# RyanXLi/OneshotDet

Hardware: AMD Instinct MI355X
Metric: images/sec/GPU fwd+bwd, 800x1024 target + 127x127 query, bs=8; 1->8 GPU scaling (higher is better)
Workload: dtype bf16; 1 GPU; BASELINE.json configs[2]: bs=8/GPU, 800x1024 target + 127x127 query, bf16 MFMA convs, forward (two R-50-FPN backbones, query pooling, correlation, FCOS head, training proposals) + FCOS loss + backward (stem/layer1 frozen) + gradient all-reduce + SGD(momentum) + weight repack; global_batch=8, parallelism=dp1: one rank, no collective anywhere in the step, world_size=1

## Files before the change

oneshotdet_amd/_lib.py:

```python
import ctypes as C
import os

_HERE = os.path.dirname(os.path.abspath(__file__))
LIB_PATH = os.environ.get("OSD_LIB_PATH") or os.path.join(_HERE, "lib", "liboneshotdet_hip.so")

OSD_F32, OSD_BF16 = 0, 1
ABI_VERSION = 4
ACT_NONE, ACT_RELU, ACT_EXP_SCALE = 0, 1, 2
RES_NONE, RES_SAME, RES_UP2X, RES_DOWN2X = 0, 1, 2, 3
GN_SPLITS = 64


class ConvDesc(C.Structure):
    _fields_ = [(n, C.c_int32) for n in (
        "dtype", "n", "h", "w", "cin", "in_stride_n", "in_stride_h", "in_stride_w", "ho", "wo", "cout", "r", "s",
        "stride_h", "stride_w", "pad_h", "pad_w", "w_rows", "out_stride", "res_mode", "res_h", "res_w", "res_stride",
        "act")] + [("act_scale", C.c_float), ("relu_in", C.c_int32), ("algo", C.c_int32), ("reserved0", C.c_int32),
                   ("ordered_ws", C.c_void_p), ("ordered_ws_bytes", C.c_int64)]


_p, _i, _f, _i64 = C.c_void_p, C.c_int, C.c_float, C.c_int64

SIGNATURES = {
    "osd_last_error_string": (C.c_char_p, []),
# ... 79 lines not shown
    "osd_box_decode": (_i, [_p, _p, _p, _p, _p, _p, _p, _i, _i, _i, _i, _p, _f, _f, _p, _f, _i, _p]),
    "osd_append_gt_boxes": (_i, [_p, _p, _p, _p, _p, _p, _p, _p, _i, _i, _i, _p]),
    "osd_proposals_sort_nms": (_i, [_p, _p, _i, _i, _i, _p, _p, _i, _i, _f, _i, _i, _p, _p, _p, _p, _p]),
    "osd_proposals_sort_nms_hint": (_i, [_p, _p, _i, _i, _i, _p, _p, _i, _i, _f, _i, _i, _i, _p, _p, _p, _p, _p, _p]),
    "osd_proposals_workspace_bytes": (_i64, [_i, _i, _i, _i]),
    "osd_box_match_sample": (_i, [_p, _p, _p, _p, _p, _p, _i, _i, _i, _i, _f, _f, _p, _p, _p, _p, _p, _p, _p, _p, _p]),
    "osd_box_loss": (_i, [_p, _p, _p, _p, _i, _i, _i, _f, _f, _p, _p, _i, _i, _p]),
    "osd_voc_match": (_i, [_p, _p, _p, _p, _p, _p, _p, _p, _i, _i, _i, _f, _p, _p, _p]),
    "osd_voc_curves": (_i, [_p, _p, _p, _i, _p, _p, _p]),
    "osd_voc_ap": (_i, [_p, _p, _p, _p, _p, _i, _i, _p, _p]),
    "osd_coco_match": (_i, [_p, _p, _p, _p, _p, _p, _i, _i, _i, _p, _i, _p, _i, _p, _p, _p, _p]),
    "osd_groupnorm_act_rois_bwd": (_i, [_p, _p, _p, _p, _p, _p, _p, _p, _p, _i, _i, _i, _i, _f, _f, _i, _i, _i, _i, _p]),
    "osd_rois_sum": (_i, [_p, _p, _i, _i, _i64, _i, _p]),
    "osd_roi_pool_levels_bwd": (_i, [_i, _p, _p, _p, _p, _p, _p, _p, _i, _i, _i, _i, _i, _i, _i, _p]),
    "osd_image_transform": (_i, [_p, _i, _i, _i, _i, _i, _i, _p, _p, _p, _i, _i, _i, _i, _i, _i, _i, _p, _p]),
    "osd_image_transform_workspace_bytes": (_i64, [_i, _i, _i, _i]),
    "osd_image_transform_batch": (_i, [_i, _p, _p, _p, _p, _p, _p, _i, _p, _p, _p, _i, _i, _i, _i, _i, _i, _i, _p, _p]),
}

BOX_CLS_CE, BOX_CLS_FOCAL, BOX_CLS_MSE = 0, 1, 2
SIGNATURES_BOX_MODES = {
    "osd_box_loss_opt": (_i, [_p, _p, _p, _p, _i, _i, _i, _f, _f, _p, _p, _i, _i, _i, _f, _f, _p]),
    "osd_box_decode_opt": (_i, [_p, _p, _p, _p, _p, _p, _p, _i, _i, _i, _i, _p, _f, _f, _p, _f, _i, _i, _p]),
}

BOX_CLS_L1, BOX_CLS_CXE = 3, 4
SOFT_LABEL_DISCRETE, SOFT_LABEL_LINEAR, SOFT_LABEL_TRANS_LINEAR, SOFT_LABEL_TRANS_4TH_LINEAR = 0, 1, 2, 3
SIGNATURES_SOFT_LABELS = {
    "osd_box_match_sample_soft": (_i, [_p, _p, _p, _p, _p, _p, _i, _i, _i, _i, _f, _f, _p, _p, _p, _p, _p, _p, _p, _p, _i, _p, _p, _p]),
    "osd_box_loss_soft": (_i, [_p, _p, _p, _p, _i, _i, _i, _f, _f, _p, _p, _i, _i, _p, _i, _p]),
}

SIGNATURES_NEG_SUPPORT = {
    "osd_box_loss_neg_support": (_i, [_p, _p, _p, _p, _p, _i, _i, _i, _f, _f, _f, _f, _p, _p, _p, _i, _i, _p]),
}

SIGNATURES_SOLVER = {
    "osd_solver_set": (_i, [_p, _f, _i, _p]),
    "osd_sgd_momentum_multi_dev": (_i, [_p, _p, _i, _p, _p, _p, _p, _f, _p]),
    "osd_sgd_momentum_pack_multi_dev": (_i, [_p, _p, _i, _p, _p, _p, _p, _p, _i, _p, _f, _i, _p]),
}

SIGNATURES_CLASS_SWEEP = {
    "osd_class_sweep_group": (_i, []),
    "osd_correlate_levels_sweep": (_i, [_i, _p, _p, _p, _p, _i, _i, _i, _i, _p]),
    "osd_roi_pool_levels_sweep": (_i, [_i, _p, _p, _p, _p, _p, _p, _p, _i, _i, _i, _i, _i, _i, _i, _p, _i, _p]),
}

SIGNATURES_GALLERY = {
    "osd_correlate_levels_gallery": (_i, [_i, _p, _p, _p, _p, _p, _i, _i, _i, _i, _i, _p]),
    "osd_groupnorm_act_rois_gallery": (_i, [_p, _p, _p, _p, _p, _p, _i, _i, _i, _i, _f, _f, _i, _i, _i, _i, _i, _p]),
}

_lib = None


class OsdError(RuntimeError):
    pass


def load():
    global _lib
    if _lib is not None:
        return _lib
    if not os.path.exists(LIB_PATH):
        raise OsdError("liboneshotdet_hip.so not built (%s missing): run `python -m oneshotdet_amd.build` or "
                       "__graft_entry__.build(); there is no CPU/eager fallback" % LIB_PATH)
    import torch
    lib = C.CDLL(LIB_PATH)
    for name, (res, args) in (list(SIGNATURES.items()) + list(SIGNATURES_BOX_MODES.items()) + list(SIGNATURES_SOFT_LABELS.items())
                              + list(SIGNATURES_NEG_SUPPORT.items()) + list(SIGNATURES_SOLVER.items())
                              + list(SIGNATURES_CLASS_SWEEP.items()) + list(SIGNATURES_GALLERY.items())):
        fn = getattr(lib, name)
        fn.restype = res
        fn.argtypes = args
    if lib.osd_abi_version() != ABI_VERSION:
        raise OsdError("%s reports ABI %d, this binding is written for ABI %d: rebuild it (`python -m oneshotdet_amd.build`)"
                       % (LIB_PATH, lib.osd_abi_version(), ABI_VERSION))
    _lib = lib
    return lib


def check(rc, what=""):
    if rc != 0:
        msg = load().osd_last_error_string()
        err = OsdError("%s failed (%d): %s" % (what, rc, msg.decode() if msg else "?"))
        err.code = rc
        raise err


def call(name, *args):
    lib = load()
    check(getattr(lib, name)(*args), name)
```

oneshotdet_amd/build.py:

```python
import os
import subprocess
import sys

HERE = os.path.dirname(os.path.abspath(__file__))
CSRC = os.path.join(HERE, "csrc")
LIBDIR = os.path.join(HERE, "lib")
TAG = os.environ.get("OSD_BUILD_TAG", "")
LIB = os.path.join(LIBDIR, "liboneshotdet_hip%s.so" % ("_" + TAG if TAG else ""))
SOURCES = ["osd_error.hip", "conv_igemm.hip", "conv_igemm_dma.hip", "conv_igemm_sp.hip", "conv_pred.hip", "conv_px.hip", "conv_wgrad.hip", "conv_wgrad_sk.hip", "backward.hip", "groupnorm_onepass.hip", "loss.hip", "elementwise.hip", "proposals.hip", "box_head.hip", "transforms.hip", "box_train.hip", "evaluation.hip", "query_avgpool.hip", "class_sweep.hip", "gallery.hip"]
HIPCC = os.environ.get("HIPCC", "/opt/rocm/bin/hipcc")
FLAGS = ["--offload-arch=gfx950", "-O3", "-fPIC", "-std=c++17", "-Wno-unused-result"] + os.environ.get("OSD_BUILD_FLAGS", "").split()


def _stale(target, deps):
    if not os.path.exists(target):
        return True
    t = os.path.getmtime(target)
    return any(os.path.getmtime(d) > t for d in deps)


def build_library(force=False, verbose=True):
    os.makedirs(LIBDIR, exist_ok=True)
    objdir = os.path.join(LIBDIR, "obj" + ("_" + TAG if TAG else ""))
    os.makedirs(objdir, exist_ok=True)
    headers = sorted(os.path.join(CSRC, f) for f in os.listdir(CSRC) if f.endswith(".h")) + [os.path.join(os.path.dirname(HERE), "include", h) for h in ("oneshotdet_hip.h", "oneshotdet_hip_box_modes.h", "oneshotdet_hip_soft_labels.h", "oneshotdet_hip_neg_support.h", "oneshotdet_hip_solver.h", "oneshotdet_hip_class_sweep.h", "oneshotdet_hip_gallery.h")]
    keep = set(src.replace(".hip", ".o") for src in SOURCES)
    for f in os.listdir(objdir):
        if f.endswith(".o") and f not in keep:
            os.remove(os.path.join(objdir, f))
    objs, procs = [], []
    for src in SOURCES:
        s = os.path.join(CSRC, src)
        o = os.path.join(objdir, src.replace(".hip", ".o"))
        objs.append(o)
        if force or _stale(o, [s] + headers):
            cmd = [HIPCC] + FLAGS + ["-c", s, "-o", o]
            if verbose:
                print(" ".join(cmd), flush=True)
            procs.append((src, subprocess.Popen(cmd, stdout=subprocess.PIPE, stderr=subprocess.STDOUT)))
    for src, p in procs:
        out, _ = p.communicate()
        if p.returncode != 0:
            sys.stderr.write(out.decode())
            raise RuntimeError("hipcc failed on %s" % src)
    if force or procs or _stale(LIB, objs):
        cmd = [HIPCC, "--offload-arch=gfx950", "-shared", "-fPIC", "-o", LIB] + objs
        if verbose:
            print(" ".join(cmd), flush=True)
        subprocess.check_call(cmd)
    return LIB


if __name__ == "__main__":
    print(build_library(force="--force" in sys.argv))
```

oneshotdet_amd/csrc/backward.hip:

```cpp
#include "osd_common.h"
#include "conv_params.h"

namespace {

constexpr int kMaxBlocks = 2048;
inline int grid_for(long long work, int threads) {
  long long b = (work + threads - 1) / threads;
  if (b < 1) b = 1;
  return (int)(b > kMaxBlocks ? kMaxBlocks : b);
}

template <typename T> struct Chunk;
template <> struct Chunk<float> {
  static constexpr int N = 4;
  float v[4];
  __device__ __forceinline__ void load(const float* p) {
    const float4 t = *reinterpret_cast<const float4*>(p);
    v[0] = t.x; v[1] = t.y; v[2] = t.z; v[3] = t.w;
  }
  __device__ __forceinline__ void store(float* p) const { *reinterpret_cast<float4*>(p) = make_float4(v[0], v[1], v[2], v[3]); }
};
template <> struct Chunk<__bf16> {
  static constexpr int N = 8;
  float v[8];
  __device__ __forceinline__ void load(const __bf16* p) {
    const bf16x8 t = *reinterpret_cast<const bf16x8*>(p);
#pragma unroll
    for (int i = 0; i < 8; ++i) v[i] = (float)t[i];
  }
  __device__ __forceinline__ void store(__bf16* p) const {
    bf16x8 t;
#pragma unroll
    for (int i = 0; i < 8; ++i) t[i] = (__bf16)v[i];
    *reinterpret_cast<bf16x8*>(p) = t;
  }
};

template <typename T>
__global__ void pack_dgrad_weight_kernel(const float* __restrict__ w, const float* __restrict__ scale, T* __restrict__ dst,
                                         int cout, int cin, int R, int S, int rows, int cout_pad, int src_orsi) {
  const long long total = (long long)rows * R * S * cout_pad;
  for (long long i = blockIdx.x * (long long)blockDim.x + threadIdx.x; i < total; i += (long long)gridDim.x * blockDim.x) {
    const int co = (int)(i % cout_pad);
    long long t = i / cout_pad;
    const int s = (int)(t % S); t /= S;
    const int r = (int)(t % R);
    const int ci = (int)(t / R);
    float v = 0.f;
    if (co < cout && ci < cin) {
      v = src_orsi ? w[(((size_t)co * R + (R - 1 - r)) * S + (S - 1 - s)) * cin + ci]
                   : w[(((size_t)co * cin + ci) * R + (R - 1 - r)) * S + (S - 1 - s)];
      if (scale) v *= scale[co];
    }
    dst[i] = from_f32<T>(v);
// ... 93 lines not shown
      for (int j = 0; j < (64 * CPW) / 256; ++j) {
        const int idx = threadIdx.x + 256 * j;
        const int ci = ci0 + idx / CPW, cc = (idx % CPW) * EP;
        if (ci >= e.rows) continue;
        T* o = out + (((size_t)ci * e.R + rr) * e.S + ss) * e.kpad + co0 + cc;
        if constexpr (sizeof(T) == 2) {
          bf16x8 v;
#pragma unroll
          for (int q = 0; q < 8; ++q) v[q] = (__bf16)big[cc + q][idx / CPW];
          *reinterpret_cast<bf16x8*>(o) = v;
        } else {
          *reinterpret_cast<f32x4*>(o) = f32x4{big[cc][idx / CPW], big[cc + 1][idx / CPW], big[cc + 2][idx / CPW], big[cc + 3][idx / CPW]};
        }
      }
    }
    return;
  }
  __shared__ float tile[32][33];
  const int tx = threadIdx.x & 31, ty = threadIdx.x >> 5;
  const int tci = (e.rows + 31) / 32, tco = (e.kpad + 31) / 32;
  const int ntiles = e.R * e.S * tci * tco;
  for (int t = blockIdx.x - e.first_block; t < ntiles; t += e.n_blocks) {
    const int cot = t % tco;
    int u = t / tco;
    const int cit = u % tci; u /= tci;
    const int s = u % e.S, r = u / e.S;
    const int co0 = cot * 32, ci0 = cit * 32;
    __syncthreads();
#pragma unroll
    for (int j = 0; j < 4; ++j) {
      const int co = co0 + ty + 8 * j, ci = ci0 + tx;
      float v = 0.f;
      if (co < e.cout && ci < e.cin) {
        v = w[(((size_t)co * e.R + (e.R - 1 - r)) * e.S + (e.S - 1 - s)) * e.cin + ci];
        if (sc) v *= sc[co];
      }
      tile[ty + 8 * j][tx] = v;
    }
    __syncthreads();
#pragma unroll
    for (int j = 0; j < 4; ++j) {
      const int ci = ci0 + ty + 8 * j, co = co0 + tx;
      if (ci < e.rows && co < e.kpad) out[(((size_t)ci * e.R + r) * e.S + s) * e.kpad + co] = from_f32<T>(tile[tx][ty + 8 * j]);
    }
  }
}

struct SgdEntry {
  long long off, numel;
  float lr_mult, wd;
  int first_block, n_blocks;
};

__device__ __forceinline__ float sgd_update(float w, float g, float b, float wd, float momentum, float step, int first, float& m) {
  const float d = __builtin_fmaf(wd, w, g);
  m = first ? d : __builtin_fmaf(momentum, b, d);
  return __builtin_fmaf(-step, m, w);
}

struct alignas(8) SolverBlock { float lr; int first_step; };
static_assert(sizeof(SolverBlock) == 8, "solver block layout (oneshotdet_hip_solver.h)");

__global__ void __launch_bounds__(64) solver_set_kernel(SolverBlock* __restrict__ block, float lr, int first_step) {
  if (blockIdx.x == 0 && threadIdx.x == 0) { block->lr = lr; block->first_step = first_step; }
}

__device__ __forceinline__ void sgd_multi_body(const SgdEntry* __restrict__ table, const int* __restrict__ block_entry,
                                               float* __restrict__ p, const float* __restrict__ g,
                                               float* __restrict__ buf, float lr, float momentum, int first) {
  const SgdEntry e = table[block_entry[blockIdx.x]];
  const float step = lr * e.lr_mult;
  const long long stride = (long long)e.n_blocks * blockDim.x;
  const long long tid = (long long)(blockIdx.x - e.first_block) * blockDim.x + threadIdx.x;
  const long long n4 = (e.off & 3) == 0 ? (e.numel >> 2) : 0;
  f32x4* p4 = reinterpret_cast<f32x4*>(p + e.off);
  const f32x4* g4 = reinterpret_cast<const f32x4*>(g + e.off);
  f32x4* b4 = reinterpret_cast<f32x4*>(buf + e.off);
  for (long long i = tid; i < n4; i += stride) {
    const f32x4 w = p4[i], gr = g4[i];
    f32x4 bb = f32x4{0.f, 0.f, 0.f, 0.f};
    if (!first) bb = b4[i];
    f32x4 m, o;
#pragma unroll
    for (int k = 0; k < 4; ++k) { float mk; o[k] = sgd_update(w[k], gr[k], bb[k], e.wd, momentum, step, first, mk); m[k] = mk; }
    b4[i] = m;
    p4[i] = o;
  }
  for (long long i = n4 * 4 + tid; i < e.numel; i += stride) {
    const long long k = e.off + i;
    const float w = p[k];
    float m;
    const float o = sgd_update(w, g[k], first ? 0.f : buf[k], e.wd, momentum, step, first, m);
    buf[k] = m;
    p[k] = o;
  }
}

__global__ void __launch_bounds__(256) sgd_multi_kernel(const SgdEntry* __restrict__ table, const int* __restrict__ block_entry,
                                                        float* __restrict__ p, const float* __restrict__ g,
                                                        float* __restrict__ buf, float lr, float momentum, int first) {
  sgd_multi_body(table, block_entry, p, g, buf, lr, momentum, first);
}

__global__ void __launch_bounds__(256) sgd_multi_dev_kernel(const SgdEntry* __restrict__ table, const int* __restrict__ block_entry,
                                                            float* __restrict__ p, const float* __restrict__ g,
                                                            float* __restrict__ buf, const SolverBlock* __restrict__ solver,
                                                            float momentum) {
  const SolverBlock s = *solver;
  sgd_multi_body(table, block_entry, p, g, buf, s.lr, momentum, s.first_step);
}

struct SgdPackEntry {
  long long off, numel;
  float lr_mult, wd;
// ... 376 lines not shown
}

#define OSD_STREAM(s) reinterpret_cast<hipStream_t>(s)
#define OSD_DISPATCH_DTYPE(dtype, CALL_F32, CALL_BF16)                            \
  do {                                                                           \
    if ((dtype) == OSD_F32) { CALL_F32; }                                        \
    else if ((dtype) == OSD_BF16) { CALL_BF16; }                                 \
    else return osd_fail(OSD_ERR_INVALID_ARG, "bad dtype %d", (int)(dtype));     \
  } while (0)

extern "C" int osd_pack_conv_weight_dgrad(const float* w, const float* scale, void* dst, int cout, int cin, int r, int s,
                                          int rows, int cout_pad, int src_orsi, int dtype, void* stream) {
  if (!w || !dst || rows < cin || cout_pad < cout) return osd_fail(OSD_ERR_INVALID_ARG, "pack_dgrad: bad args");
  const int g = grid_for((long long)rows * r * s * cout_pad, 256);
  OSD_DISPATCH_DTYPE(dtype,
      hipLaunchKernelGGL(pack_dgrad_weight_kernel<float>, dim3(g), dim3(256), 0, OSD_STREAM(stream), w, scale, (float*)dst, cout, cin, r, s, rows, cout_pad, src_orsi),
      hipLaunchKernelGGL(pack_dgrad_weight_kernel<__bf16>, dim3(g), dim3(256), 0, OSD_STREAM(stream), w, scale, (__bf16*)dst, cout, cin, r, s, rows, cout_pad, src_orsi));
  return osd_check_launch("pack_dgrad_weight");
}

extern "C" int osd_pack_multi(const void* table, const int32_t* block_entry, int n_blocks, const float* src,
                              const float* scales, void* dst, int dgrad, int dtype, void* stream) {
  if (!table || !block_entry || !src || !dst) return osd_fail(OSD_ERR_INVALID_ARG, "pack_multi: null argument");
  if (n_blocks <= 0) return OSD_OK;
  OSD_DISPATCH_DTYPE(dtype,
      hipLaunchKernelGGL(pack_multi_kernel<float>, dim3(n_blocks), dim3(256), 0, OSD_STREAM(stream), (const PackEntry*)table, block_entry, src, scales, (float*)dst, dgrad),
      hipLaunchKernelGGL(pack_multi_kernel<__bf16>, dim3(n_blocks), dim3(256), 0, OSD_STREAM(stream), (const PackEntry*)table, block_entry, src, scales, (__bf16*)dst, dgrad));
  return osd_check_launch("pack_multi");
}

extern "C" int osd_sgd_momentum_multi(const void* table, const int32_t* block_entry, int n_blocks, float* params,
                                      const float* grads, float* momentum_buf, float lr, float momentum, int first_step,
                                      void* stream) {
  if (!table || !block_entry || !params || !grads || !momentum_buf) return osd_fail(OSD_ERR_INVALID_ARG, "sgd: null argument");
  if (n_blocks <= 0) return OSD_OK;
  hipLaunchKernelGGL(sgd_multi_kernel, dim3(n_blocks), dim3(256), 0, OSD_STREAM(stream), (const SgdEntry*)table, block_entry,
                     params, grads, momentum_buf, lr, momentum, first_step);
  return osd_check_launch("sgd_multi");
}

extern "C" int osd_sgd_momentum_pack_multi(const void* table, const int32_t* block_entry, int n_blocks, float* params,
                                           float* grads, float* momentum_buf, const float* scales, void* packed, int dtype,
                                           float lr, float momentum, int first_step, int zero_grads, void* stream) {
  if (!table || !block_entry || !params || !grads || !momentum_buf || !packed) return osd_fail(OSD_ERR_INVALID_ARG, "sgd_pack: null argument");
  if (n_blocks <= 0) return OSD_OK;
  OSD_DISPATCH_DTYPE(dtype,
      hipLaunchKernelGGL(sgd_pack_multi_kernel<float>, dim3(n_blocks), dim3(256), 0, OSD_STREAM(stream), (const SgdPackEntry*)table, block_entry,
                         params, grads, momentum_buf, scales, (float*)packed, lr, momentum, first_step, zero_grads),
      hipLaunchKernelGGL(sgd_pack_multi_kernel<__bf16>, dim3(n_blocks), dim3(256), 0, OSD_STREAM(stream), (const SgdPackEntry*)table, block_entry,
                         params, grads, momentum_buf, scales, (__bf16*)packed, lr, momentum, first_step, zero_grads));
  return osd_check_launch("sgd_pack_multi");
}

static int solver_block_ok(const void* block, const char* who) {
  if (!block) return osd_fail(OSD_ERR_INVALID_ARG, "%s: null solver block", who);
  if (reinterpret_cast<uintptr_t>(block) & 7) return osd_fail(OSD_ERR_INVALID_ARG, "%s: the solver block %p is not 8-byte aligned", who, block);
  return OSD_OK;
}

extern "C" int osd_solver_set(void* block, float lr, int first_step, void* stream) {
  if (const int rc = solver_block_ok(block, "solver_set")) return rc;
  hipLaunchKernelGGL(solver_set_kernel, dim3(1), dim3(64), 0, OSD_STREAM(stream), (SolverBlock*)block, lr, first_step);
  return osd_check_launch("solver_set");
}

extern "C" int osd_sgd_momentum_multi_dev(const void* table, const int32_t* block_entry, int n_blocks, float* params,
                                          const float* grads, float* momentum_buf, const void* solver_block, float momentum,
                                          void* stream) {
  if (!table || !block_entry || !params || !grads || !momentum_buf) return osd_fail(OSD_ERR_INVALID_ARG, "sgd_dev: null argument");
  if (const int rc = solver_block_ok(solver_block, "sgd_dev")) return rc;
  if (n_blocks <= 0) return OSD_OK;
  hipLaunchKernelGGL(sgd_multi_dev_kernel, dim3(n_blocks), dim3(256), 0, OSD_STREAM(stream), (const SgdEntry*)table, block_entry,
                     params, grads, momentum_buf, (const SolverBlock*)solver_block, momentum);
  return osd_check_launch("sgd_multi_dev");
}

extern "C" int osd_sgd_momentum_pack_multi_dev(const void* table, const int32_t* block_entry, int n_blocks, float* params,
                                               float* grads, float* momentum_buf, const float* scales, void* packed, int dtype,
                                               const void* solver_block, float momentum, int zero_grads, void* stream) {
  if (!table || !block_entry || !params || !grads || !momentum_buf || !packed) return osd_fail(OSD_ERR_INVALID_ARG, "sgd_pack_dev: null argument");
  if (const int rc = solver_block_ok(solver_block, "sgd_pack_dev")) return rc;
  if (n_blocks <= 0) return OSD_OK;
  OSD_DISPATCH_DTYPE(dtype,
      hipLaunchKernelGGL(sgd_pack_multi_dev_kernel<float>, dim3(n_blocks), dim3(256), 0, OSD_STREAM(stream), (const SgdPackEntry*)table, block_entry,
                         params, grads, momentum_buf, scales, (float*)packed, (const SolverBlock*)solver_block, momentum, zero_grads),
      hipLaunchKernelGGL(sgd_pack_multi_dev_kernel<__bf16>, dim3(n_blocks), dim3(256), 0, OSD_STREAM(stream), (const SgdPackEntry*)table, block_entry,
                         params, grads, momentum_buf, scales, (__bf16*)packed, (const SolverBlock*)solver_block, momentum, zero_grads));
  return osd_check_launch("sgd_pack_multi_dev");
}

extern "C" int osd_unpack_wgrad(const float* dw_packed, const float* scale, float* grad_oihw, int cout, int cin, int r, int s,
                                int accumulate, void* stream) {
  if (!dw_packed || !grad_oihw) return osd_fail(OSD_ERR_INVALID_ARG, "unpack_wgrad: null argument");
  hipLaunchKernelGGL(unpack_wgrad_kernel, dim3(grid_for((long long)cout * cin * r * s, 256)), dim3(256), 0, OSD_STREAM(stream),
                     dw_packed, scale, grad_oihw, cout, cin, r, s, accumulate);
  return osd_check_launch("unpack_wgrad");
}

extern "C" int osd_scatter2x(const void* src, const void* mask, const void* addend, void* dst, int n, int h, int w, int ho,
                             int wo, int c, int dtype, void* stream) {
  const int e = dtype == OSD_BF16 ? 8 : 4;
  if (!src || !dst || c % e) return osd_fail(OSD_ERR_INVALID_ARG, "scatter2x: bad args");
  const int g = grid_for((long long)n * h * w * (c / e), 256);
  OSD_DISPATCH_DTYPE(dtype,
      hipLaunchKernelGGL(scatter2x_kernel<float>, dim3(g), dim3(256), 0, OSD_STREAM(stream), (const float*)src, (const float*)mask, (const float*)addend, (float*)dst, n, h, w, ho, wo, c),
      hipLaunchKernelGGL(scatter2x_kernel<__bf16>, dim3(g), dim3(256), 0, OSD_STREAM(stream), (const __bf16*)src, (const __bf16*)mask, (const __bf16*)addend, (__bf16*)dst, n, h, w, ho, wo, c));
  return osd_check_launch("scatter2x");
}

extern "C" int osd_add_mask(const void* a, const void* b, const void* mask, void* out, int64_t numel, int dtype, void* stream) {
  const int e = dtype == OSD_BF16 ? 8 : 4;
// ... 686 lines not shown
```

oneshotdet_amd/train_update.py:

```python
import os

import torch

from . import streams

from . import ops
from .ops import PackedConv


class Update(object):
    def _build_pack_tables(self):
        import numpy as np
        mult = 64 if self.dtype == torch.bfloat16 else 16
        tr = [c for c in self.convs.values() if c.trainable]
        scale_off, scales = {}, []
        off = 0
        for c in tr:
            if c.bn_scale is not None:
                scale_off[c.name] = off
                scales.append(c.bn_scale)
                off += c.cout
        self._flat_scale = torch.cat(scales) if scales else torch.zeros(1, device=self.device)
        base = self.flat_w.data_ptr()
        self._pack = {}
        for form in (0, 1):
            entries, dst_off = [], 0
            for c in tr:
                if form == 0:
                    rows, kpad = ops._round_up(c.cout, 16), ops._round_up(c.cin, mult)
                else:
                    rows, kpad = ops._round_up(c.cin, 16), ops._round_up(c.cout, mult)
                numel = rows * c.r * c.s * kpad
                nb = max(1, min(64, (numel + 256 * 16 - 1) // (256 * 16)))
                entries.append(dict(c=c, src=(c.w.data_ptr() - base) // 4, dst=dst_off, scale=scale_off.get(c.name, -1), rows=rows,
                                    kpad=kpad, nb=nb, numel=numel))
                dst_off += (numel + 63) // 64 * 64
            flat = torch.zeros(dst_off, device=self.device, dtype=self.dtype)
            tables = {}
            for bucket in self.exchange.ranges:
                sub = [e for e in entries if self._bucket_of(e["c"].w) == bucket]
                if not sub:
                    continue
                tab = np.zeros((len(sub), 7), dtype=np.int64)
                blocks = []
                for i, e in enumerate(sub):
                    c = e["c"]
                    tab[i, 0:3] = (e["src"], e["dst"], e["scale"])
                    tab[i, 3:7] = np.frombuffer(np.array([c.cout, c.cin, c.r, c.s, e["rows"], e["kpad"], len(blocks), e["nb"]],
                                                         dtype=np.int32).tobytes(), dtype=np.int64)
                    blocks += [i] * e["nb"]
                tables[bucket] = dict(table=torch.from_numpy(tab).to(self.device),
                                      blocks=torch.tensor(blocks, dtype=torch.int32, device=self.device), n=len(blocks))
            self._pack[form] = dict(flat=flat, tables=tables)
            if form == 0:
                self._pack_fwd_entry = {id(e["c"]): e for e in entries}
            for e in entries:
                c = e["c"]
                view = flat[e["dst"]:e["dst"] + e["numel"]].view(e["rows"], c.r, c.s, e["kpad"])
                if form == 0:
                    cout_store = ops._round_up(c.cout, 4)
                    if c.has_bias and c.cout % 16 == 0:
                        bias = c.b
                    else:
                        bias = torch.zeros(ops._round_up(cout_store, 16), device=self.device, dtype=torch.float32)
                        if c.bn_shift is not None:
                            bias[:c.cout] = c.bn_shift
                    c.pc = PackedConv(view, bias, c.cout, cout_store, e["rows"], e["kpad"], c.r, c.s, cin_real=c.cin)
                else:
                    zb = torch.zeros(ops._round_up(c.cin, 16), device=self.device, dtype=torch.float32)
                    c.pd = PackedConv(view, zb, c.cin, c.cin, e["rows"], e["kpad"], c.r, c.s, cin_real=c.cout)
        self._padded_bias = {}
        for c in tr:
            if c.has_bias and c.cout % 16 != 0:
                self._padded_bias.setdefault(self._bucket_of(c.w), []).append(c)

    def repack(self, buckets=None, forms=(0, 1)):
        for c in self.convs.values():
            if not c.trainable and c.pc is None:
                c.pc = ops.pack_conv(self._frozen_sd[c.name + ".weight"], bn=None if c.bn_scale is None else tuple(
                    self._frozen_sd[c.name.replace("conv", "bn").replace("downsample.0", "downsample.1") + k]
                    for k in (".weight", ".bias", ".running_mean", ".running_var")), dtype=self.dtype,
                    stem=c.name.endswith("stem.conv1"))
        if not hasattr(self, "_pack"):
            self._build_pack_tables()
        for bucket in (self.exchange.ranges if buckets is None else buckets):
            for form in forms:
                pk = self._pack[form]
                tb = pk["tables"].get(bucket)
                if tb is not None:
                    ops._lib.call("osd_pack_multi", ops._ptr(tb["table"]), ops._ptr(tb["blocks"]), tb["n"], ops._ptr(self.flat_w),
                                  ops._ptr(self._flat_scale), ops._ptr(pk["flat"]), form, ops._dt(pk["flat"]), ops._stream())
            for c in self._padded_bias.get(bucket, ()):
                c.pc.bias[:c.cout] = c.b

    def _build_sgd_table(self, weights, biases):
        import numpy as np
        base = self.flat_w.data_ptr()
        conv_of = {c.w.data_ptr(): c for c in self.convs.values() if c.trainable}
        rows = {name: [] for name in self.exchange.ranges}
        for group, lr_mult, wd in ((weights, 1.0, self.weight_decay), (biases, 2.0, 0.0)):
            for t in group:
                rows[self._bucket_of(t)].append(((t.data_ptr() - base) // 4, t.numel(), lr_mult, wd, conv_of.get(t.data_ptr())))
        fuse = os.environ.get("OSD_NO_FUSED_REPACK", "0") == "0"
        tables = {}
        for name, rs in rows.items():
            if not rs:
                continue
            fused = fuse
            tab = np.zeros((len(rs), 8 if fused else 4), dtype=np.int64)
            blocks = []
            for i, (off, n, lm, wd, c) in enumerate(rs):
                nb = max(1, min(64, (n + 256 * 16 - 1) // (256 * 16)))
                tab[i, 0], tab[i, 1] = off, n
                tab[i, 2] = np.frombuffer(np.array([lm, wd], dtype=np.float32).tobytes(), dtype=np.int64)[0]
                tab[i, 3] = np.frombuffer(np.array([len(blocks), nb], dtype=np.int32).tobytes(), dtype=np.int64)[0]
                if fused:
                    tab[i, 4] = tab[i, 5] = -1
                    if c is not None:
                        e = self._pack_fwd_entry[id(c)]
                        cout = n // (c.cin * c.r * c.s)
                        assert e["kpad"] >= c.cin and cout * c.cin * c.r * c.s == n, (name, i, e["kpad"], c.cin, n)
                        assert 0 <= e["dst"] and e["dst"] + cout * c.r * c.s * e["kpad"] <= self._pack[0]["flat"].numel(), (name, i)
                        tab[i, 4], tab[i, 5] = e["dst"], e["scale"]
                        tab[i, 6:8] = np.frombuffer(np.array([c.cin, c.r * c.s, e["kpad"], 0], dtype=np.int32).tobytes(), dtype=np.int64)
                blocks += [i] * nb
            tables[name] = dict(table=torch.from_numpy(tab).to(self.device), fused=fused,
                                blocks=torch.tensor(blocks, dtype=torch.int32, device=self.device), n=len(blocks))
        self._sgd = dict(tables=tables, buf=torch.zeros_like(self.flat_w), steps=0)

    def _update_bucket(self, name):
        sg = self._sgd
        tb = sg["tables"].get(name)
        fused = tb is not None and tb["fused"]
        if fused and self._dev_update:
            pk = self._pack[0]["flat"]
            ops.sgd_momentum_pack_multi_dev(tb["table"], tb["blocks"], tb["n"], self.flat_w, self.flat_g, sg["buf"], self._flat_scale,
                                            pk, self._solver, self.momentum, self.consume_grads)
            if self.consume_grads:
                self._zeroed.add(name)
        elif fused:
            pk = self._pack[0]["flat"]
            ops._lib.call("osd_sgd_momentum_pack_multi", ops._ptr(tb["table"]), ops._ptr(tb["blocks"]), tb["n"],
                          ops._ptr(self.flat_w), ops._ptr(self.flat_g), ops._ptr(sg["buf"]), ops._ptr(self._flat_scale), ops._ptr(pk),
                          ops._dt(pk), float(self.lr), float(self.momentum), int(sg["steps"] == 0), int(self.consume_grads), ops._stream())
            if self.consume_grads:
                self._zeroed.add(name)
        elif tb is not None and self._dev_update:
            ops.sgd_momentum_multi_dev(tb["table"], tb["blocks"], tb["n"], self.flat_w, self.flat_g, sg["buf"], self._solver,
                                       self.momentum)
        elif tb is not None:
            ops._lib.call("osd_sgd_momentum_multi", ops._ptr(tb["table"]), ops._ptr(tb["blocks"]), tb["n"],
                          ops._ptr(self.flat_w), ops._ptr(self.flat_g), ops._ptr(sg["buf"]), float(self.lr),
                          float(self.momentum), int(sg["steps"] == 0), ops._stream())
        self.repack([name], forms=(1,) if fused else (0, 1))
        self._updated.add(name)

    def optimizer_step(self):
        self._scheduled_lr()
        if self.opt is not None:
            self.opt.step()
            self.repack()
            self._sgd["steps"] += 1
            return
        if self._overlap:
            main = streams.current()
            main.wait_stream(self.ustream)
            if self.exchange.comm is not None:
                main.wait_stream(self.exchange.comm)
        for name in self.exchange.ranges:
            if name not in self._updated:
                self._update_bucket(name)
        self._end_of_update()
        self._sgd["steps"] += 1

    def _end_of_update(self):
        self._updated = set()
        self._grads_clean = bool(self.consume_grads and self._zeroed >= set(self._sgd["tables"]))
        self._zeroed = set()
```

Before: 784.4 images/sec.

## Fuse SGD update with forward and dgrad weight repacks in one kernel

Adds an update_forms kernel that applies SGD momentum to each conv weight and, in the same pass, writes both the forward packed layout and the flipped/transposed data-gradient packed layout through a shared-memory tile. It also writes padded predictor bias copies. This is meant to remove the separate dgrad repack pass, which re-read the weights and launched extra kernels. The cost is a more complex kernel that does a tile transpose through shared memory, and small tensors go through a second launch.

```diff
diff --git a/include/oneshotdet_hip_update.h b/include/oneshotdet_hip_update.h
--- /dev/null
+++ b/include/oneshotdet_hip_update.h
@@ -0,0 +1,22 @@
+#ifndef ONESHOTDET_HIP_UPDATE_H
+#define ONESHOTDET_HIP_UPDATE_H
+
+#include "oneshotdet_hip_solver.h"
+
+#ifdef __cplusplus
+extern "C" {
+#endif
+
+int osd_sgd_momentum_update_forms(const void* table, const int32_t* block_entry, int n_blocks, float* params, float* grads,
+                                  float* momentum_buf, const float* scales, void* packed, void* packed_dgrad, int dtype, float lr,
+                                  float momentum, int first_step, int zero_grads, void* stream);
+
+int osd_sgd_momentum_update_forms_solver(const void* table, const int32_t* block_entry, int n_blocks, float* params, float* grads,
+                                      float* momentum_buf, const float* scales, void* packed, void* packed_dgrad, int dtype,
+                                      const void* solver_block, float momentum, int zero_grads, void* stream);
+
+#ifdef __cplusplus
+}
+#endif
+
+#endif
diff --git a/oneshotdet_amd/_lib.py b/oneshotdet_amd/_lib.py
--- a/oneshotdet_amd/_lib.py
+++ b/oneshotdet_amd/_lib.py
@@ -155,6 +155,11 @@
     "osd_groupnorm_act_rois_gallery": (_i, [_p, _p, _p, _p, _p, _p, _i, _i, _i, _i, _f, _f, _i, _i, _i, _i, _i, _p]),
 }
 
+SIGNATURES_UPDATE = {
+    "osd_sgd_momentum_update_forms": (_i, [_p, _p, _i, _p, _p, _p, _p, _p, _p, _i, _f, _f, _i, _i, _p]),
+    "osd_sgd_momentum_update_forms_solver": (_i, [_p, _p, _i, _p, _p, _p, _p, _p, _p, _i, _p, _f, _i, _p]),
+}
+
 _lib = None
 
 
@@ -173,7 +178,8 @@
     lib = C.CDLL(LIB_PATH)
     for name, (res, args) in (list(SIGNATURES.items()) + list(SIGNATURES_BOX_MODES.items()) + list(SIGNATURES_SOFT_LABELS.items())
                               + list(SIGNATURES_NEG_SUPPORT.items()) + list(SIGNATURES_SOLVER.items())
-                              + list(SIGNATURES_CLASS_SWEEP.items()) + list(SIGNATURES_GALLERY.items())):
+                              + list(SIGNATURES_CLASS_SWEEP.items()) + list(SIGNATURES_GALLERY.items())
+                              + list(SIGNATURES_UPDATE.items())):
         fn = getattr(lib, name)
         fn.restype = res
         fn.argtypes = args
diff --git a/oneshotdet_amd/build.py b/oneshotdet_amd/build.py
--- a/oneshotdet_amd/build.py
+++ b/oneshotdet_amd/build.py
@@ -7,7 +7,7 @@
 LIBDIR = os.path.join(HERE, "lib")
 TAG = os.environ.get("OSD_BUILD_TAG", "")
 LIB = os.path.join(LIBDIR, "liboneshotdet_hip%s.so" % ("_" + TAG if TAG else ""))
-SOURCES = ["osd_error.hip", "conv_igemm.hip", "conv_igemm_dma.hip", "conv_igemm_sp.hip", "conv_pred.hip", "conv_px.hip", "conv_wgrad.hip", "conv_wgrad_sk.hip", "backward.hip", "groupnorm_onepass.hip", "loss.hip", "elementwise.hip", "proposals.hip", "box_head.hip", "transforms.hip", "box_train.hip", "evaluation.hip", "query_avgpool.hip", "class_sweep.hip", "gallery.hip"]
+SOURCES = ["osd_error.hip", "conv_igemm.hip", "conv_igemm_dma.hip", "conv_igemm_sp.hip", "conv_pred.hip", "conv_px.hip", "conv_wgrad.hip", "conv_wgrad_sk.hip", "backward.hip", "groupnorm_onepass.hip", "loss.hip", "elementwise.hip", "proposals.hip", "box_head.hip", "transforms.hip", "box_train.hip", "evaluation.hip", "query_avgpool.hip", "class_sweep.hip", "gallery.hip", "update_forms.hip"]
 HIPCC = os.environ.get("HIPCC", "/opt/rocm/bin/hipcc")
 FLAGS = ["--offload-arch=gfx950", "-O3", "-fPIC", "-std=c++17", "-Wno-unused-result"] + os.environ.get("OSD_BUILD_FLAGS", "").split()
 
@@ -23,7 +23,7 @@
     os.makedirs(LIBDIR, exist_ok=True)
     objdir = os.path.join(LIBDIR, "obj" + ("_" + TAG if TAG else ""))
     os.makedirs(objdir, exist_ok=True)
-    headers = sorted(os.path.join(CSRC, f) for f in os.listdir(CSRC) if f.endswith(".h")) + [os.path.join(os.path.dirname(HERE), "include", h) for h in ("oneshotdet_hip.h", "oneshotdet_hip_box_modes.h", "oneshotdet_hip_soft_labels.h", "oneshotdet_hip_neg_support.h", "oneshotdet_hip_solver.h", "oneshotdet_hip_class_sweep.h", "oneshotdet_hip_gallery.h")]
+    headers = sorted(os.path.join(CSRC, f) for f in os.listdir(CSRC) if f.endswith(".h")) + [os.path.join(os.path.dirname(HERE), "include", h) for h in ("oneshotdet_hip.h", "oneshotdet_hip_box_modes.h", "oneshotdet_hip_soft_labels.h", "oneshotdet_hip_neg_support.h", "oneshotdet_hip_solver.h", "oneshotdet_hip_class_sweep.h", "oneshotdet_hip_gallery.h", "oneshotdet_hip_update.h")]
     keep = set(src.replace(".hip", ".o") for src in SOURCES)
     for f in os.listdir(objdir):
         if f.endswith(".o") and f not in keep:
diff --git a/oneshotdet_amd/csrc/backward.hip b/oneshotdet_amd/csrc/backward.hip
--- a/oneshotdet_amd/csrc/backward.hip
+++ b/oneshotdet_amd/csrc/backward.hip
@@ -1,5 +1,6 @@
 #include "osd_common.h"
 #include "conv_params.h"
+#include "sgd_update.h"
 
 namespace {
 
@@ -199,14 +200,6 @@
   int first_block, n_blocks;
 };
 
-__device__ __forceinline__ float sgd_update(float w, float g, float b, float wd, float momentum, float step, int first, float& m) {
-  const float d = __builtin_fmaf(wd, w, g);
-  m = first ? d : __builtin_fmaf(momentum, b, d);
-  return __builtin_fmaf(-step, m, w);
-}
-
-struct alignas(8) SolverBlock { float lr; int first_step; };
-static_assert(sizeof(SolverBlock) == 8, "solver block layout (oneshotdet_hip_solver.h)");
 
 __global__ void __launch_bounds__(64) solver_set_kernel(SolverBlock* __restrict__ block, float lr, int first_step) {
   if (blockIdx.x == 0 && threadIdx.x == 0) { block->lr = lr; block->first_step = first_step; }
@@ -689,11 +682,6 @@
   return osd_check_launch("sgd_pack_multi");
 }
 
-static int solver_block_ok(const void* block, const char* who) {
-  if (!block) return osd_fail(OSD_ERR_INVALID_ARG, "%s: null solver block", who);
-  if (reinterpret_cast<uintptr_t>(block) & 7) return osd_fail(OSD_ERR_INVALID_ARG, "%s: the solver block %p is not 8-byte aligned", who, block);
-  return OSD_OK;
-}
 
 extern "C" int osd_solver_set(void* block, float lr, int first_step, void* stream) {
   if (const int rc = solver_block_ok(block, "solver_set")) return rc;
diff --git a/oneshotdet_amd/csrc/sgd_update.h b/oneshotdet_amd/csrc/sgd_update.h
--- /dev/null
+++ b/oneshotdet_amd/csrc/sgd_update.h
@@ -0,0 +1,17 @@
+#pragma once
+#include "osd_common.h"
+
+__device__ __forceinline__ float sgd_update(float w, float g, float b, float wd, float momentum, float step, int first, float& m) {
+  const float d = __builtin_fmaf(wd, w, g);
+  m = first ? d : __builtin_fmaf(momentum, b, d);
+  return __builtin_fmaf(-step, m, w);
+}
+
+struct alignas(8) SolverBlock { float lr; int first_step; };
+static_assert(sizeof(SolverBlock) == 8, "solver block layout (oneshotdet_hip_solver.h)");
+
+static inline int solver_block_ok(const void* block, const char* who) {
+  if (!block) return osd_fail(OSD_ERR_INVALID_ARG, "%s: null solver block", who);
+  if (reinterpret_cast<uintptr_t>(block) & 7) return osd_fail(OSD_ERR_INVALID_ARG, "%s: the solver block %p is not 8-byte aligned", who, block);
+  return OSD_OK;
+}
diff --git a/oneshotdet_amd/csrc/update_forms.hip b/oneshotdet_amd/csrc/update_forms.hip
--- /dev/null
+++ b/oneshotdet_amd/csrc/update_forms.hip
@@ -0,0 +1,239 @@
+#include "sgd_update.h"
+#include "../../include/oneshotdet_hip_update.h"
+
+#define OSD_STREAM(s) reinterpret_cast<hipStream_t>(s)
+
+namespace {
+
+struct UpdateFormsEntry {
+  long long off, numel;
+  float lr_mult, wd;
+  int first_block, n_blocks;
+  long long dst_off;
+  long long scale_off;
+  long long ddst_off;
+  long long copy_addr;
+  int cout, cin;
+  int R, S;
+  int kpad, dkpad;
+  int drows, pad_;
+};
+static_assert(sizeof(UpdateFormsEntry) == 96, "update table layout (oneshotdet_hip_update.h)");
+
+template <typename T> struct Rounded;
+template <> struct Rounded<float> { static __device__ __forceinline__ float of(float v) { return v; } };
+template <> struct Rounded<__bf16> { static __device__ __forceinline__ float of(float v) { return (float)(__bf16)v; } };
+
+template <typename T>
+__device__ __forceinline__ void update_forms_body(const UpdateFormsEntry* __restrict__ table, const int* __restrict__ block_entry,
+                                                  float* __restrict__ p, float* __restrict__ g, float* __restrict__ buf,
+                                                  const float* __restrict__ scales, T* __restrict__ packed, T* __restrict__ dpacked,
+                                                  float lr, float momentum, int first, int zero_grads) {
+  __shared__ float tile[64][65];
+  const UpdateFormsEntry e = table[block_entry[blockIdx.x]];
+  const float step = lr * e.lr_mult;
+  const int tid = threadIdx.x;
+
+  if (e.dst_off < 0) {
+    const long long stride = (long long)e.n_blocks * blockDim.x;
+    const long long t0 = (long long)(blockIdx.x - e.first_block) * blockDim.x + tid;
+    const long long n4 = (e.off & 3) == 0 ? (e.numel >> 2) : 0;
+    f32x4* p4 = reinterpret_cast<f32x4*>(p + e.off);
+    f32x4* g4 = reinterpret_cast<f32x4*>(g + e.off);
+    f32x4* b4 = reinterpret_cast<f32x4*>(buf + e.off);
+    float* copy = reinterpret_cast<float*>(e.copy_addr);
+    for (long long i = t0; i < n4; i += stride) {
+      const f32x4 w = p4[i], gr = g4[i];
+      f32x4 bb = f32x4{0.f, 0.f, 0.f, 0.f};
+      if (!first) bb = b4[i];
+      f32x4 m, o;
+#pragma unroll
+      for (int k = 0; k < 4; ++k) { float mk; o[k] = sgd_update(w[k], gr[k], bb[k], e.wd, momentum, step, first, mk); m[k] = mk; }
+      b4[i] = m;
+      p4[i] = o;
+      if (zero_grads) g4[i] = f32x4{0.f, 0.f, 0.f, 0.f};
+      if (copy) {
+#pragma unroll
+        for (int k = 0; k < 4; ++k) copy[i * 4 + k] = o[k];
+      }
+    }
+    for (long long i = n4 * 4 + t0; i < e.numel; i += stride) {
+      const long long k = e.off + i;
+      float m;
+      const float o = sgd_update(p[k], g[k], first ? 0.f : buf[k], e.wd, momentum, step, first, m);
+      buf[k] = m;
+      p[k] = o;
+      if (zero_grads) g[k] = 0.f;
+      if (copy) copy[i] = o;
+    }
+    return;
+  }
+
+  constexpr int EP = 16 / (int)sizeof(T);
+  constexpr int CPW = 64 / EP;
+  const int RS = e.R * e.S;
+  const int tci = (e.cin + 63) >> 6, tco = (e.cout + 63) >> 6;
+  const int nunits = tco * RS * tci;
+  const bool vec = (e.off & 3) == 0 && (e.cin & 3) == 0 && (e.kpad & 3) == 0 && (e.dst_off & 3) == 0;
+  const bool dvec = e.dkpad % EP == 0 && e.ddst_off % EP == 0;
+  float* pw = p + e.off;
+  float* pg = g + e.off;
+  float* pb = buf + e.off;
+  const float* sc = e.scale_off >= 0 ? scales + e.scale_off : nullptr;
+  T* fwd = packed + e.dst_off;
+
+  for (int u = blockIdx.x - e.first_block; u < nunits; u += e.n_blocks) {
+    const int cit = u % tci;
+    const int v = u / tci;
+    const int tap = v % RS, cot = v / RS;
+    const int co0 = cot << 6, ci0 = cit << 6;
+    const int r = tap / e.S, s = tap - r * e.S;
+    const int ftap = (e.R - 1 - r) * e.S + (e.S - 1 - s);
+    __syncthreads();
+    if (vec) {
+      const int lco = tid >> 4, lci = (tid & 15) << 2;
+      const int ci = ci0 + lci;
+      f32x4 w[4], gr[4], bb[4];
+      bool in[4];
+#pragma unroll
+      for (int j = 0; j < 4; ++j) {
+        const int co = co0 + lco + 16 * j;
+        in[j] = co < e.cout && ci < e.cin;
+        if (in[j]) {
+          const size_t i = ((size_t)co * RS + tap) * e.cin + ci;
+          w[j] = *reinterpret_cast<const f32x4*>(pw + i);
+          gr[j] = *reinterpret_cast<const f32x4*>(pg + i);
+          bb[j] = first ? f32x4{0.f, 0.f, 0.f, 0.f} : *reinterpret_cast<const f32x4*>(pb + i);
+        }
+      }
+#pragma unroll
+      for (int j = 0; j < 4; ++j) {
+        if (!in[j]) continue;
+        const int co = co0 + lco + 16 * j;
+        const size_t i = ((size_t)co * RS + tap) * e.cin + ci;
+        f32x4 m, o;
+#pragma unroll
+        for (int k = 0; k < 4; ++k) { float mk; o[k] = sgd_update(w[j][k], gr[j][k], bb[j][k], e.wd, momentum, step, first, mk); m[k] = mk; }
+        *reinterpret_cast<f32x4*>(pb + i) = m;
+        *reinterpret_cast<f32x4*>(pw + i) = o;
+        if (zero_grads) *reinterpret_cast<f32x4*>(pg + i) = f32x4{0.f, 0.f, 0.f, 0.f};
+        const float f = sc ? sc[co] : 1.f;
+        f32x4 q;
+#pragma unroll
+        for (int k = 0; k < 4; ++k) q[k] = Rounded<T>::of(o[k] * f);
+        T* d = fwd + ((size_t)co * RS + tap) * e.kpad + ci;
+        if constexpr (sizeof(T) == 2) {
+          bf16x4 h;
+#pragma unroll
+          for (int k = 0; k < 4; ++k) h[k] = (__bf16)q[k];
+          *reinterpret_cast<bf16x4*>(d) = h;
+        } else {
+          *reinterpret_cast<f32x4*>(d) = q;
+        }
+        float* trow = &tile[lco + 16 * j][lci];
+        trow[0] = q[0]; trow[1] = q[1]; trow[2] = q[2]; trow[3] = q[3];
+      }
+    } else {
+#pragma unroll 4
+      for (int j = 0; j < 16; ++j) {
+        const int idx = tid + 256 * j;
+        const int lco = idx >> 6, lci = idx & 63;
+        const int co = co0 + lco, ci = ci0 + lci;
+        if (co >= e.cout || ci >= e.cin) continue;
+        const size_t i = ((size_t)co * RS + tap) * e.cin + ci;
+        float m;
+        const float o = sgd_update(pw[i], pg[i], first ? 0.f : pb[i], e.wd, momentum, step, first, m);
+        pb[i] = m;
+        pw[i] = o;
+        if (zero_grads) pg[i] = 0.f;
+        const float q = Rounded<T>::of(o * (sc ? sc[co] : 1.f));
+        fwd[((size_t)co * RS + tap) * e.kpad + ci] = from_f32<T>(q);
+        tile[lco][lci] = q;
+      }
+    }
+    __syncthreads();
+    if (e.ddst_off < 0) continue;
+    T* dg = dpacked + e.ddst_off;
+#pragma unroll
+    for (int j = 0; j < (64 * CPW) / 256; ++j) {
+      const int idx = tid + 256 * j;
+      const int lci = idx / CPW, cc = (idx % CPW) * EP;
+      const int ci = ci0 + lci, co = co0 + cc;
+      if (ci >= e.cin || co >= e.cout) continue;
+      T* o = dg + ((size_t)ci * RS + ftap) * e.dkpad + co;
+      if (dvec && co + EP <= e.cout) {
+        if constexpr (sizeof(T) == 2) {
+          bf16x8 h;
+#pragma unroll
+          for (int q = 0; q < 8; ++q) h[q] = (__bf16)tile[cc + q][lci];
+          *reinterpret_cast<bf16x8*>(o) = h;
+        } else {
+          *reinterpret_cast<f32x4*>(o) = f32x4{tile[cc][lci], tile[cc + 1][lci], tile[cc + 2][lci], tile[cc + 3][lci]};
+        }
+      } else {
+#pragma unroll
+        for (int q = 0; q < EP; ++q)
+          if (co + q < e.cout) o[q] = from_f32<T>(tile[cc + q][lci]);
+      }
+    }
+  }
+}
+
+template <typename T>
+__global__ void __launch_bounds__(256) update_forms_kernel(const UpdateFormsEntry* __restrict__ table, const int* __restrict__ block_entry,
+                                                           float* __restrict__ p, float* __restrict__ g, float* __restrict__ buf,
+                                                           const float* __restrict__ scales, T* __restrict__ packed,
+                                                           T* __restrict__ dpacked, float lr, float momentum, int first,
+                                                           int zero_grads) {
+  update_forms_body<T>(table, block_entry, p, g, buf, scales, packed, dpacked, lr, momentum, first, zero_grads);
+}
+
+template <typename T>
+__global__ void __launch_bounds__(256) update_forms_solver_kernel(const UpdateFormsEntry* __restrict__ table, const int* __restrict__ block_entry,
+                                                               float* __restrict__ p, float* __restrict__ g, float* __restrict__ buf,
+                                                               const float* __restrict__ scales, T* __restrict__ packed,
+                                                               T* __restrict__ dpacked, const SolverBlock* __restrict__ solver,
+                                                               float momentum, int zero_grads) {
+  const SolverBlock s = *solver;
+  update_forms_body<T>(table, block_entry, p, g, buf, scales, packed, dpacked, s.lr, momentum, s.first_step, zero_grads);
+}
+
+int args_ok(const char* who, const void* table, const int32_t* block_entry, int n_blocks, const float* params, const float* grads,
+            const float* momentum_buf, const void* packed, const void* packed_dgrad, int dtype) {
+  if (!table || !block_entry || !params || !grads || !momentum_buf) return osd_fail(OSD_ERR_INVALID_ARG, "%s: null argument", who);
+  if (!packed || !packed_dgrad) return osd_fail(OSD_ERR_INVALID_ARG, "%s: null packed buffer (forward %p, data gradient %p)", who, packed, packed_dgrad);
+  if (n_blocks < 0) return osd_fail(OSD_ERR_INVALID_ARG, "%s: n_blocks %d < 0", who, n_blocks);
+  if (dtype != OSD_F32 && dtype != OSD_BF16) return osd_fail(OSD_ERR_INVALID_ARG, "%s: bad dtype %d", who, dtype);
+  return OSD_OK;
+}
+
+}
+
+extern "C" int osd_sgd_momentum_update_forms(const void* table, const int32_t* block_entry, int n_blocks, float* params, float* grads,
+                                             float* momentum_buf, const float* scales, void* packed, void* packed_dgrad, int dtype,
+                                             float lr, float momentum, int first_step, int zero_grads, void* stream) {
+  if (const int rc = args_ok("sgd_update_forms", table, block_entry, n_blocks, params, grads, momentum_buf, packed, packed_dgrad, dtype)) return rc;
+  if (n_blocks == 0) return OSD_OK;
+  if (dtype == OSD_F32)
+    hipLaunchKernelGGL(update_forms_kernel<float>, dim3(n_blocks), dim3(256), 0, OSD_STREAM(stream), (const UpdateFormsEntry*)table, block_entry,
+                       params, grads, momentum_buf, scales, (float*)packed, (float*)packed_dgrad, lr, momentum, first_step, zero_grads);
+  else
+    hipLaunchKernelGGL(update_forms_kernel<__bf16>, dim3(n_blocks), dim3(256), 0, OSD_STREAM(stream), (const UpdateFormsEntry*)table, block_entry,
+                       params, grads, momentum_buf, scales, (__bf16*)packed, (__bf16*)packed_dgrad, lr, momentum, first_step, zero_grads);
+  return osd_check_launch("sgd_update_forms");
+}
+
+extern "C" int osd_sgd_momentum_update_forms_solver(const void* table, const int32_t* block_entry, int n_blocks, float* params, float* grads,
+                                                 float* momentum_buf, const float* scales, void* packed, void* packed_dgrad, int dtype,
+                                                 const void* solver_block, float momentum, int zero_grads, void* stream) {
+  if (const int rc = args_ok("sgd_update_forms_solver", table, block_entry, n_blocks, params, grads, momentum_buf, packed, packed_dgrad, dtype)) return rc;
+  if (const int rc = solver_block_ok(solver_block, "sgd_update_forms_solver")) return rc;
+  if (n_blocks == 0) return OSD_OK;
+  if (dtype == OSD_F32)
+    hipLaunchKernelGGL(update_forms_solver_kernel<float>, dim3(n_blocks), dim3(256), 0, OSD_STREAM(stream), (const UpdateFormsEntry*)table, block_entry,
+                       params, grads, momentum_buf, scales, (float*)packed, (float*)packed_dgrad, (const SolverBlock*)solver_block, momentum, zero_grads);
+  else
+    hipLaunchKernelGGL(update_forms_solver_kernel<__bf16>, dim3(n_blocks), dim3(256), 0, OSD_STREAM(stream), (const UpdateFormsEntry*)table, block_entry,
+                       params, grads, momentum_buf, scales, (__bf16*)packed, (__bf16*)packed_dgrad, (const SolverBlock*)solver_block, momentum, zero_grads);
+  return osd_check_launch("sgd_update_forms_solver");
+}
diff --git a/oneshotdet_amd/train_update.py b/oneshotdet_amd/train_update.py
--- a/oneshotdet_amd/train_update.py
+++ b/oneshotdet_amd/train_update.py
@@ -54,6 +54,8 @@
             self._pack[form] = dict(flat=flat, tables=tables)
             if form == 0:
                 self._pack_fwd_entry = {id(e["c"]): e for e in entries}
+            else:
+                self._pack_dgrad_entry = {id(e["c"]): e for e in entries}
             for e in entries:
                 c = e["c"]
                 view = flat[e["dst"]:e["dst"] + e["numel"]].view(e["rows"], c.r, c.s, e["kpad"])
@@ -97,19 +99,18 @@
         import numpy as np
         base = self.flat_w.data_ptr()
         conv_of = {c.w.data_ptr(): c for c in self.convs.values() if c.trainable}
+        padded = {c.b.data_ptr(): c for cs in self._padded_bias.values() for c in cs}
         rows = {name: [] for name in self.exchange.ranges}
         for group, lr_mult, wd in ((weights, 1.0, self.weight_decay), (biases, 2.0, 0.0)):
             for t in group:
-                rows[self._bucket_of(t)].append(((t.data_ptr() - base) // 4, t.numel(), lr_mult, wd, conv_of.get(t.data_ptr())))
+                rows[self._bucket_of(t)].append(((t.data_ptr() - base) // 4, t.numel(), lr_mult, wd,
+                                                 conv_of.get(t.data_ptr()), padded.get(t.data_ptr())))
         fuse = os.environ.get("OSD_NO_FUSED_REPACK", "0") == "0"
-        tables = {}
-        for name, rs in rows.items():
-            if not rs:
-                continue
-            fused = fuse
+        both = fuse and os.environ.get("OSD_NO_FUSED_DGRAD_PACK", "0") == "0"
+        def pack_table(name, rs, fused):
             tab = np.zeros((len(rs), 8 if fused else 4), dtype=np.int64)
             blocks = []
-            for i, (off, n, lm, wd, c) in enumerate(rs):
+            for i, (off, n, lm, wd, c, _) in enumerate(rs):
                 nb = max(1, min(64, (n + 256 * 16 - 1) // (256 * 16)))
                 tab[i, 0], tab[i, 1] = off, n
                 tab[i, 2] = np.frombuffer(np.array([lm, wd], dtype=np.float32).tobytes(), dtype=np.int64)[0]
@@ -124,14 +125,82 @@
                         tab[i, 4], tab[i, 5] = e["dst"], e["scale"]
                         tab[i, 6:8] = np.frombuffer(np.array([c.cin, c.r * c.s, e["kpad"], 0], dtype=np.int32).tobytes(), dtype=np.int64)
                 blocks += [i] * nb
-            tables[name] = dict(table=torch.from_numpy(tab).to(self.device), fused=fused,
-                                blocks=torch.tensor(blocks, dtype=torch.int32, device=self.device), n=len(blocks))
+            return dict(table=torch.from_numpy(tab).to(self.device), fused=fused, forms=False,
+                        blocks=torch.tensor(blocks, dtype=torch.int32, device=self.device), n=len(blocks))
+
+        tables = {}
+        for name, rs in rows.items():
+            if not rs:
+                continue
+            if both:
+                big = [r for r in rs if r[4] is not None or r[5] is not None]
+                small = [r[:4] + (None, None) for r in rs if r[4] is None and r[5] is None]
+                tables[name] = self._update_forms_table(name, big) if any(r[4] is not None for r in big) else pack_table(name, rs, True)
+                if tables[name]["forms"]:
+                    tables[name]["small"] = pack_table(name, small, True) if small else None
+                continue
+            tables[name] = pack_table(name, rs, fuse)
         self._sgd = dict(tables=tables, buf=torch.zeros_like(self.flat_w), steps=0)
+
+    def _update_forms_table(self, name, rs):
+        import numpy as np
+
+        def i32(*v):
+            return np.frombuffer(np.array(v, dtype=np.int32).tobytes(), dtype=np.int64)
+
+        tab = np.zeros((len(rs), 12), dtype=np.int64)
+        blocks, keep = [], []
+        for i, (off, n, lm, wd, c, pred) in enumerate(rs):
+            nb = max(1, min(64, (n + 256 * 16 - 1) // (256 * 16)))
+            tab[i, 0], tab[i, 1] = off, n
+            tab[i, 2] = np.frombuffer(np.array([lm, wd], dtype=np.float32).tobytes(), dtype=np.int64)[0]
+            tab[i, 3] = i32(len(blocks), nb)[0]
+            tab[i, 4] = tab[i, 5] = tab[i, 6] = -1
+            if c is not None:
+                e, d = self._pack_fwd_entry[id(c)], self._pack_dgrad_entry[id(c)]
+                taps = c.r * c.s
+                assert c.cout * taps * c.cin == n, (name, i, c.cout, taps, c.cin, n)
+                assert e["kpad"] >= c.cin and e["rows"] >= c.cout, (name, i, e["rows"], e["kpad"])
+                assert 0 <= e["dst"] and e["dst"] + c.cout * taps * e["kpad"] <= self._pack[0]["flat"].numel(), (name, i)
+                assert d["kpad"] >= c.cout and d["rows"] >= c.cin, (name, i, d["rows"], d["kpad"])
+                assert 0 <= d["dst"] and d["dst"] + c.cin * taps * d["kpad"] <= self._pack[1]["flat"].numel(), (name, i)
+                assert e["scale"] == d["scale"], (name, i)
+                tab[i, 4], tab[i, 5], tab[i, 6] = e["dst"], e["scale"], d["dst"]
+                tab[i, 8:12] = i32(c.cout, c.cin, c.r, c.s, e["kpad"], d["kpad"], d["rows"], 0)
+            elif pred is not None:
+                assert pred.pc.bias.dtype == torch.float32 and pred.pc.bias.numel() >= n == pred.cout, (name, i)
+                tab[i, 7] = pred.pc.bias.data_ptr()
+                keep.append(pred.pc.bias)
+            blocks += [i] * nb
+        return dict(table=torch.from_numpy(tab).to(self.device), fused=True, forms=True, keep=keep,
+                    blocks=torch.tensor(blocks, dtype=torch.int32, device=self.device), n=len(blocks))
 
     def _update_bucket(self, name):
         sg = self._sgd
         tb = sg["tables"].get(name)
         fused = tb is not None and tb["fused"]
+        if fused and tb["forms"]:
+            pk, pd = self._pack[0]["flat"], self._pack[1]["flat"]
+            sm = tb["small"]
+            if sm is not None and self._dev_update:
+                ops.sgd_momentum_pack_multi_dev(sm["table"], sm["blocks"], sm["n"], self.flat_w, self.flat_g, sg["buf"], self._flat_scale,
+                                                pk, self._solver, self.momentum, self.consume_grads)
+            elif sm is not None:
+                ops._lib.call("osd_sgd_momentum_pack_multi", ops._ptr(sm["table"]), ops._ptr(sm["blocks"]), sm["n"],
+                              ops._ptr(self.flat_w), ops._ptr(self.flat_g), ops._ptr(sg["buf"]), ops._ptr(self._flat_scale), ops._ptr(pk),
+                              ops._dt(pk), float(self.lr), float(self.momentum), int(sg["steps"] == 0), int(self.consume_grads), ops._stream())
+            head = (ops._ptr(tb["table"]), ops._ptr(tb["blocks"]), tb["n"], ops._ptr(self.flat_w), ops._ptr(self.flat_g),
+                    ops._ptr(sg["buf"]), ops._ptr(self._flat_scale), ops._ptr(pk), ops._ptr(pd), ops._dt(pk))
+            if self._dev_update:
+                ops._lib.call("osd_sgd_momentum_update_forms_solver", *head, ops._ptr(self._solver), float(self.momentum),
+                              int(self.consume_grads), ops._stream())
+            else:
+                ops._lib.call("osd_sgd_momentum_update_forms", *head, float(self.lr), float(self.momentum), int(sg["steps"] == 0),
+                              int(self.consume_grads), ops._stream())
+            if self.consume_grads:
+                self._zeroed.add(name)
+            self._updated.add(name)
+            return
         if fused and self._dev_update:
             pk = self._pack[0]["flat"]
             ops.sgd_momentum_pack_multi_dev(tb["table"], tb["blocks"], tb["n"], self.flat_w, self.flat_g, sg["buf"], self._flat_scale,
```

Result: no change. 784.7 images/sec, median of 3 (+0.0%).
